# kywind/real2sim-eval

Measured on AMD Instinct MI355X. Metric: sim env-steps/sec (phys+render) per node at 32 envs, higher is better.
Workload: dtype f32

## Files before the change

include/r2s_physics.h:

```cpp
#ifndef R2S_PHYSICS_H
#define R2S_PHYSICS_H

#include <stddef.h>
#include <stdint.h>
#include "r2s_raster.h"

#ifdef __cplusplus
extern "C" {
#endif

typedef struct R2SPhysParams {
    float dt;
    float dashpot_damping;
    float drag_damping;
    float spring_Y_min;
    float spring_Y_max;
    float collision_dist;
    float collide_elas, collide_fric;
    float collide_eef_elas, collide_eef_fric;
    float collide_self_elas, collide_self_fric;
    int32_t reverse_z;
    int32_t self_collision;
    int32_t use_pusher;
    int32_t num_substeps;
// ... 101 lines not shown
    char kernel[192];
} R2SFlavourOut;
int r2s_phys_debug_pick_flavour(const R2SFlavourIn* in, R2SFlavourOut* out);
int r2s_phys_debug_flavour_input(R2SPhys* h, R2SFlavourIn* out);

int r2s_phys_last_flavour_ex(R2SPhys* h, R2SFlavourOut* out);
int r2s_phys_check_fault(R2SPhys* h, r2s_stream_t stream);

int r2s_phys_set_tuning(R2SPhys* h, int chains, int mesh_defer);
int r2s_phys_set_resident(R2SPhys* h, int on);
int r2s_phys_set_pf(R2SPhys* h, int on);
int r2s_phys_side_stream(int32_t k, r2s_stream_t* out);

int r2s_phys_layout_stats(R2SPhys* h, int64_t* out);

void r2s_phys_set_timing(R2SPhys* h, int enable);
int r2s_phys_last_step_ms(R2SPhys* h, float* ms, int32_t* kernels);

#ifdef __cplusplus
}
#endif
#endif
```

real2sim-eval_amd/csrc/physics.hip:

```cpp

#include "r2s_common.h"
#include <rocprim/rocprim.hpp>
#include "../../include/r2s_physics.h"
#include "physics_flavour.h"
#include <algorithm>
#include <array>
#include <climits>
#include <cmath>
#include <cstdlib>
#include <mutex>
#include <vector>
#include <functional>

namespace {

constexpr int SLICE = 64;

constexpr int GROUP = 4;
constexpr int TPB = 256;
constexpr int GRID_DIM = 128;
constexpr int GRID_CELL_BITS = 21;
constexpr float MESH_MAX_DIST = 0.02f;
constexpr float WIND_THRESHOLD = 0.6f;
constexpr float NEAR_PAD = 0.03f;
// ... 1 lines not shown
struct PhysDev {
    int N, E, n_sub;
    int nb, cb;
    int e0, ne;
    const int* slice_off;
    const int* slice_deg;
    const int* slice_int;
    const uint2* adj_idx;
    const float4* adj_k;
    const float4* adj_ir;
    const int* rslice_off;
    const int* rslice_deg;
    const int4* radj;
    const int* halo_off;
    const int* halo_ids;
    const int* perm;
    const int* inv;
    const float* masses;
    const int* masks;
    float dt, dashpot, drag_factor, rf, cd;
    float ce, cf, cee, cef, cse, csf;
    int self_collision, use_pusher;
    const int* coll_num;
    const int* coll_idx;
    int coll_cap;
    size_t par_stride;
    float4* vbc;
    float4* xbc;
    float4* vdef;
    int2* mesh_list;
// ... 103 lines not shown

struct R2SPhys {
    R2SPhysParams prm{};
    int E = 0, N = 0, S = 0, n_slices = 0, ell_len = 0;
    int nb = 0, cb = 0, halo_max = 0;
    int pb = 256, rcap = 1024;
    int coll_cap = 500;
    int words = 0;
    int n_mesh = 0, n_dyn_mesh = 0, nF = 0, nV = 0, n_dyn_pts = 0;
    std::vector<int> h_springs;
    std::vector<float> h_rest;
    std::vector<int> h_adj_spring;
    std::vector<int> h_adj_nbr;
    std::vector<int> h_adj_self;
    std::vector<int> h_adj_loc;
    std::vector<int> h_perm, h_inv, h_slice_off, h_slice_deg, h_rslice_off, h_rslice_deg, h_slice_int;
    std::vector<int> h_radj_spring, h_radj_nbr, h_radj_self;
    std::vector<int> h_mesh_map, h_face_map;
    v2f* xv[2] = {nullptr, nullptr};
    StateM state(int b) const { return {xv[b], (size_t)E * N}; }
    int cur = 0;
    int *d_slice_off = nullptr, *d_slice_deg = nullptr, *d_rslice_off = nullptr, *d_rslice_deg = nullptr, *d_slice_int = nullptr;
    unsigned short* d_adj_idx = nullptr;
    float *d_adj_k = nullptr, *d_adj_ir = nullptr;
    int4* d_radj = nullptr;
    int rell_len = 0;
    int *d_halo_off = nullptr, *d_halo_ids = nullptr, *d_perm = nullptr, *d_inv = nullptr;
    int *d_num_user = nullptr, *d_idx_user = nullptr;
    float* d_masses = nullptr;
    int* d_masks = nullptr;
    int *d_coll_num = nullptr, *d_coll_idx = nullptr, *d_max_count = nullptr;
// ... 84 lines not shown
    hipGraph_t graph_tail[MAX_CHAINS][12] = {};
    hipGraphExec_t graph_exec_tail[MAX_CHAINS][12] = {};
    int graph_head = 64;
    hipEvent_t chain_fork = nullptr, chain_join[MAX_CHAINS] = {};
    bool timing = false;
    hipEvent_t ev0 = nullptr, ev1 = nullptr;
    int last_kernels = 0;
    bool ev_pending = false;

    PhysDev dev() const
    {
        PhysDev p{};
        p.N = N; p.E = E; p.n_sub = prm.num_substeps;
        p.nb = nb; p.cb = cb; p.e0 = 0; p.ne = E;
        p.slice_off = d_slice_off; p.slice_deg = d_slice_deg; p.slice_int = d_slice_int; p.adj_idx = (const uint2*)d_adj_idx; p.adj_k = (const float4*)d_adj_k; p.adj_ir = (const float4*)d_adj_ir; p.rslice_off = d_rslice_off; p.rslice_deg = d_rslice_deg; p.radj = d_radj;
        p.halo_off = d_halo_off; p.halo_ids = d_halo_ids; p.perm = d_perm; p.inv = d_inv;
        p.masses = d_masses; p.masks = d_masks;
        p.dt = prm.dt; p.dashpot = prm.dashpot_damping; p.drag_factor = expf(-prm.dt * prm.drag_damping);
        p.rf = prm.reverse_z ? -1.f : 1.f; p.cd = prm.collision_dist;
        auto cl = [](float x, float lo, float hi) { return std::min(std::max(x, lo), hi); };
        p.ce = cl(prm.collide_elas, 0.f, 1.f); p.cf = cl(prm.collide_fric, 0.f, 2.f);
        p.cee = cl(prm.collide_eef_elas, 0.f, 1.f); p.cef = cl(prm.collide_eef_fric, 0.f, 2.f);
        p.cse = cl(prm.collide_self_elas, 0.f, 1.f); p.csf = cl(prm.collide_self_fric, 0.f, 2.f);
        p.self_collision = prm.self_collision; p.use_pusher = prm.use_pusher;
        p.coll_num = d_coll_num; p.coll_idx = d_coll_idx; p.coll_cap = coll_cap;
        p.vbc = d_vbc; p.xbc = d_xbc; p.par_stride = (size_t)E * N; p.cand_list = d_cand_list; p.cand_count = d_cand_count; p.cand_cnt_env = d_cand_count ? d_cand_count + 4 : nullptr;
        p.pf = 0; p.pf_nfin = 0; p.pf_res = d_pf_res;
        p.mesh_list = d_mesh_list; p.mesh_cnt = d_mesh_cnt; p.mesh_cap = mesh_cap; p.mesh_defer = mesh_defer; p.vdef = d_vdef; p.cand_mark = d_cand_mark; p.mesh_rec = d_mesh_rec; p.rec_cnt = d_rec_cnt; p.mq_hint = d_mq_hint;
        p.lm_c0 = lm[0]; p.lm_nc = lm[1]; p.lm_f0 = lm[2]; p.lm_f1 = lm[3]; p.lm_y = lm[4]; p.lm_mesh = lm[5]; p.lm_slot = lm[6];
        p.n_mesh = n_mesh; p.n_dyn_mesh = n_dyn_mesh; p.nF = nF; p.nV = nV; p.n_dyn_pts = n_dyn_pts;
        p.faces = d_faces; p.mesh_map = d_mesh_map; p.face_map = d_face_map; p.mesh_face_off = d_mesh_face_off;
// ... 503 lines not shown
        auto spread = [](uint64_t v) {
            v &= 0x1fffff; v = (v | v << 32) & 0x1f00000000ffffull; v = (v | v << 16) & 0x1f0000ff0000ffull;
            v = (v | v << 8) & 0x100f00f00f00f00full; v = (v | v << 4) & 0x10c30c30c30c30c3ull; v = (v | v << 2) & 0x1249249249249249ull;
            return v;
        };
        std::vector<std::pair<uint64_t, int>> code(N);
        for (int i = 0; i < N; ++i) {
            uint64_t c = 0;
            for (int k = 0; k < 3; ++k) {
                const double t = (d->init_vertices[3 * i + k] - lo[k]) / ext;
                c |= spread((uint64_t)std::min(1048575.0, std::max(0.0, t * 1048575.0))) << k;
            }
            code[i] = {c, i};
        }
        std::sort(code.begin(), code.end());
        std::vector<int> degree(N, 0);
        for (int sp = 0; sp < S; ++sp) { degree[h->h_springs[2 * sp]]++; degree[h->h_springs[2 * sp + 1]]++; }
        for (int b0 = 0; b0 < N; b0 += PB)
            std::stable_sort(code.begin() + b0, code.begin() + std::min(N, b0 + PB),
                             [&](const std::pair<uint64_t, int>& a, const std::pair<uint64_t, int>& b) { return degree[a.second] > degree[b.second]; });
        for (int i = 0; i < N; ++i) { h->h_perm[i] = code[i].second; h->h_inv[code[i].second] = i; }
    }
    TRY(dev_alloc(&h->d_perm, N)); TRY(dev_alloc(&h->d_inv, N));
    TRY(upload(h->d_perm, h->h_perm.data(), N, s)); TRY(upload(h->d_inv, h->h_inv.data(), N, s));

    std::vector<std::vector<std::pair<int, int>>> adj(N);
    for (int sp = 0; sp < S; ++sp) {
        const int a = h->h_inv[h->h_springs[2 * sp]], b = h->h_inv[h->h_springs[2 * sp + 1]];
        adj[a].push_back({b, sp});
        adj[b].push_back({a, sp});
    }
    for (auto& l : adj) std::sort(l.begin(), l.end());
    h->n_slices = (N + SL - 1) / SL;
    h->nb = (N + PB - 1) / PB;
    h->cb = (h->nb * E + 7) / 8;
    int HALO_CAP = h->rcap - PB;
    if (const char* ev = getenv("R2S_HALO_CAP")) HALO_CAP = std::min(HALO_CAP, std::max(0, atoi(ev)));
    std::vector<int> halo_off(h->nb + 1, 0), halo_ids;
    std::vector<int> slot_of(N, -1);
    std::vector<std::vector<int>> halo_of_block(h->nb);
    h->halo_max = 0;
    for (int b = 0; b < h->nb; ++b) {
        std::vector<std::pair<int, int>> cnt;
        {
            std::vector<int> refs;
            for (int i = b * PB; i < std::min(N, (b + 1) * PB); ++i)
                for (auto& nb : adj[i]) if (nb.first / PB != b) refs.push_back(nb.first);
            std::sort(refs.begin(), refs.end());
            for (size_t a = 0; a < refs.size();) {
                size_t e2 = a;
                while (e2 < refs.size() && refs[e2] == refs[a]) ++e2;
                cnt.push_back({-(int)(e2 - a), refs[a]});
                a = e2;
            }
        }
        std::sort(cnt.begin(), cnt.end());
        if ((int)cnt.size() > HALO_CAP) cnt.resize(HALO_CAP);
        std::vector<int>& hl = halo_of_block[b];
        for (auto& c : cnt) hl.push_back(c.second);
        std::sort(hl.begin(), hl.end());
        halo_off[b + 1] = halo_off[b] + (int)hl.size();
        halo_ids.insert(halo_ids.end(), hl.begin(), hl.end());
        h->halo_max = std::max(h->halo_max, (int)hl.size());
    }
    std::vector<std::vector<std::array<int, 3>>> loc(N), rem(N);
    for (int b = 0; b < h->nb; ++b) {
        const std::vector<int>& hl = halo_of_block[b];
        for (size_t k = 0; k < hl.size(); ++k) slot_of[hl[k]] = PB + (int)k;
        for (int i = b * PB; i < std::min(N, (b + 1) * PB); ++i)
            for (auto& nb : adj[i]) {
                const int j = nb.first;
                if (j / PB == b) loc[i].push_back({j, nb.second, j % PB});
                else if (slot_of[j] >= 0) loc[i].push_back({j, nb.second, slot_of[j]});
                else rem[i].push_back({j, nb.second, -1});
            }
        for (size_t k = 0; k < hl.size(); ++k) slot_of[hl[k]] = -1;
    }
    h->h_slice_int.assign(h->n_slices, 0);
    if (PB == SL)
        for (int b = 0; b < h->nb; ++b) {
            int imax = 0;
            for (int i = b * PB; i < std::min(N, (b + 1) * PB); ++i) {
                std::stable_partition(loc[i].begin(), loc[i].end(), [&](const std::array<int, 3>& a) { return a[2] < PB; });
                int ni = 0;
                for (auto& a : loc[i]) ni += a[2] < PB;
                imax = std::max(imax, ni);
            }
            imax = (imax + GROUP - 1) / GROUP * GROUP;
            h->h_slice_int[b] = imax;
            for (int i = b * PB; i < std::min(N, (b + 1) * PB); ++i) {
                int ni = 0;
                for (auto& a : loc[i]) ni += a[2] < PB;
                loc[i].insert(loc[i].begin() + ni, (size_t)(imax - ni), std::array<int, 3>{i, -1, i % PB});
// ... 1080 lines not shown
    R2S_HIP_TRY(hipGetLastError());
    return R2S_OK;
}

int r2s_phys_layout_stats(R2SPhys* h, int64_t* out )
{
    if (!h || !out) return R2S_ERR_INVALID;
    int64_t real = 0, fallback = 0;
    for (int t = 0; t < h->ell_len; ++t) if (h->h_adj_spring[t] >= 0) ++real;
    for (int t = 0; t < h->rell_len; ++t) if (h->h_radj_spring[t] >= 0) { ++real; ++fallback; }
    out[0] = h->nb; out[1] = h->halo_max; out[2] = h->ell_len + h->rell_len; out[3] = real; out[4] = fallback;
    out[5] = (int64_t)h->rcap * 24; out[6] = h->chains(); out[7] = h->cb;
    return R2S_OK;
}

void r2s_phys_set_timing(R2SPhys* h, int enable) { if (h) h->timing = enable != 0; }

int r2s_phys_last_step_ms(R2SPhys* h, float* ms, int32_t* kernels)
{
    if (!h || !ms || !h->ev_pending) return R2S_ERR_INVALID;
    R2S_HIP_TRY(hipEventSynchronize(h->ev1));
    R2S_HIP_TRY(hipEventElapsedTime(ms, h->ev0, h->ev1));
    if (kernels) *kernels = h->last_kernels;
    return R2S_OK;
}

}
```

real2sim-eval_amd/csrc/physics_resident.h:

```cpp

constexpr int RES_THREADS = 512;
constexpr int RES_NG = 2;
constexpr unsigned RES_SPIN_LIMIT = 1u << 21;
constexpr int RES_AUX_SC1 = 16;
#ifndef R2S_RES_AUXLD
#define R2S_RES_AUXLD (16 | (int)0x80000000)
#endif
#ifndef R2S_RES_PRE
#define R2S_RES_PRE 2
#endif
#ifndef R2S_RES_DELAY
#define R2S_RES_DELAY 0
#endif
constexpr int RES_AUX_LOAD = R2S_RES_AUXLD;
constexpr int RES_PRE = R2S_RES_PRE;

struct GroupRecs { v2f xy[GROUP], zz[GROUP], vv[GROUP]; };
template <int RCAP>
__device__ __forceinline__ void group_read(const AdjGroup& g, const __attribute__((address_space(3))) char* win, GroupRecs& r)
{
    typedef __attribute__((address_space(3))) const v2f lds_f2;
    const unsigned off[GROUP] = {g.idx.x & 0xffffu, g.idx.x >> 16, g.idx.y & 0xffffu, g.idx.y >> 16};
#pragma unroll
    for (int u = 0; u < GROUP; ++u) {
// ... 88 lines not shown
    const bool own = p.srv_own != 0;
    const int pl = r * 64 + lane;
    const unsigned xn = ((unsigned)p.N + 7u) & ~7u, xe = (unsigned)e * 6u * xn, xb = 3u * xn * 16u;
    const __amdgpu_buffer_rsrc_t rx = __builtin_amdgcn_make_buffer_rsrc(p.xch, 0, 0x7fffffff, 0x00020000);
    unsigned noff = 0, roff = 0;
    float sk = 0.f, sa = 0.f, m1 = 1.f, inv_m1 = 1.f;
    bool live = false;
    if (own) {
        const int b = i / SLICE, l = i - b * SLICE;
        const int srow = p.slice_off[b] / GROUP, nslot = p.slice_deg[b];
        if (pl < nslot) {
            const size_t el = (size_t)(srow + (pl / GROUP) * SLICE + l) * GROUP + (size_t)(pl % GROUP);
            const unsigned off = ((const unsigned short*)p.adj_idx)[el];
            sk = ((const float*)p.adj_k)[el]; sa = ((const float*)p.adj_ir)[el];
            const int w = (int)(off >> 3);
            const int gid = w < SLICE ? b * SLICE + w : p.halo_ids[p.halo_off[b] + (w - SLICE)];
            live = gid != i && (sk != 0.f || sa != 0.f);
            noff = (xe + (unsigned)gid) * 16u;
            roff = ((unsigned)e * (unsigned)p.N + (unsigned)gid) * (unsigned)SRV_REC + (unsigned)SRV_RES;
        }
        m1 = p.masses[i]; inv_m1 = 1.0f / m1;
    }
    f3 sx = mk(0.f, 0.f, 0.f), sv = sx;
    bool have = false;
    const unsigned k_first = k;
#ifdef R2S_PHASE_PROBE
    long long sp_acc[6] = {0, 0, 0, 0, 0, 0}, sp_t = (long long)wall_clock64();
#define R2S_SSTAMP(kk) do { const long long now_ = (long long)wall_clock64(); sp_acc[kk] += now_ - sp_t; sp_t = now_; } while (0)
#else
#define R2S_SSTAMP(kk) do { } while (0)
#endif
// ... 127 lines not shown
    const unsigned xn = ((unsigned)p.N + 7u) & ~7u;
    const unsigned xe = (unsigned)e * 6u * xn, xb = 3u * xn * 16u;
    const __amdgpu_buffer_rsrc_t rx = __builtin_amdgcn_make_buffer_rsrc(p.xch, 0, 0x7fffffff, 0x00020000);
    __attribute__((address_space(3))) char* win_w = (__attribute__((address_space(3))) char*)win_s;
    const __attribute__((address_space(3))) char* win = win_w;
    const bool finisher = wave < (n_steps == 1 ? 1 : 3);

    const int h0 = p.halo_off[b], nh = p.halo_off[b + 1] - h0, nt = 3 * nh;
    unsigned t_off[KT], t_lds[KT], pend0 = 0;
#pragma unroll
    for (int k = 0; k < KT; ++k) {
        const int t = tid + RES_THREADS * k;
        t_off[k] = 0; t_lds[k] = 0;
        if (t < nt) {
            const int pl = t / nh, r = t - pl * nh;
            const int hid = p.halo_ids[h0 + r];
            t_off[k] = (xe + (unsigned)pl * xn + (unsigned)hid) * 16u;
            t_lds[k] = (unsigned)(pl * (RCAP + 1) + B + r) * 8u;
            pend0 |= 1u << k;
            win_s[pl * (RCAP + 1) + B + r] = xv_in.p[st_at(xv_in.n, eb + (size_t)hid, pl)];
        }
    }
    if (wave < 3) win_s[wave * (RCAP + 1) + lane] = xv_in.p[st_at(xv_in.n, eb + (size_t)ic, wave)];
    const int srow = __builtin_amdgcn_readfirstlane(p.slice_off[b] / GROUP);
    const int ng = __builtin_amdgcn_readfirstlane(p.slice_deg[b] / GROUP), gi = __builtin_amdgcn_readfirstlane(p.slice_int[b] / GROUP);
    const int n_own = gi > wave ? (gi - wave + NW - 1) / NW : 0;
    const int n_all = ng > wave ? (ng - wave + NW - 1) / NW : 0, n_halo = n_all - n_own;
    AdjGroup ag_own[RES_NG], ag_halo[RES_NG];
#pragma unroll
    for (int j = 0; j < RES_NG; ++j) {
        ag_own[j].idx = make_uint2(0u, 0u); ag_own[j].k = make_float4(0.f, 0.f, 0.f, 0.f); ag_own[j].a = ag_own[j].k;
// ... 561 lines not shown
```

real2sim-eval_amd/csrc/physics_substep.h:

```cpp

typedef unsigned v4u __attribute__((ext_vector_type(4)));
constexpr unsigned PF_SENT = 0x7fc5e7a1u;
constexpr int PF_LINE = 128;
constexpr int PF_AUX_STORE = 16;
constexpr int PF_AUX_LOAD = 16 | (int)0x80000000;
__device__ __forceinline__ void resident_fault(const PhysDev& p, int code, int item, int k, unsigned a, unsigned b, unsigned c, unsigned d, unsigned e2, unsigned f)
{
    if (!p.fault) return;
    if (atomicCAS(p.fault, 0, code) == 0) {
        int* w = p.fault + 3;
        w[0] = code; w[1] = item; w[2] = k; w[3] = (int)a; w[4] = (int)b; w[5] = (int)c; w[6] = (int)d; w[7] = (int)e2; w[8] = (int)f;
    }
}
__device__ __forceinline__ bool pf_pending(v2f a) { return __float_as_uint(a.x) == PF_SENT && __float_as_uint(a.y) == PF_SENT; }
__device__ __forceinline__ void pf_mark(StateM s, size_t i)
{
    const v2f w = {__uint_as_float(PF_SENT), __uint_as_float(PF_SENT)};
    s.p[st_at(s.n, i, 0)] = w; s.p[st_at(s.n, i, 1)] = w; s.p[st_at(s.n, i, 2)] = w;
}
__device__ __forceinline__ void pf_store(const PhysDev& p, size_t ei, f3 x, f3 v, unsigned tag)
{
    const __amdgpu_buffer_rsrc_t r = __builtin_amdgcn_make_buffer_rsrc(p.pf_res, 0, 0x7fffffff, 0x00020000);
    const unsigned off = (unsigned)ei * (unsigned)PF_LINE;
    const v4u w0 = {__float_as_uint(x.x), tag, __float_as_uint(x.y), tag}, w1 = {__float_as_uint(x.z), tag, __float_as_uint(v.z), tag},
// ... 75 lines not shown
#ifdef R2S_WIN16
        typedef float v4f_ __attribute__((ext_vector_type(4)));
        typedef __attribute__((address_space(3))) const v4f_ lds_f4;
        const v4f_ xz = *(lds_f4*)(win + 2u * off[u]);
        const v2f vxy = *(lds_f2*)(win + off[u] + 2 * (RCAP * 8 + 8));
        spring_term((v2f){xz.x, xz.y}, xz.z, vxy, xz.w, xi, vi, k[u], a[u], p.dashpot, fxy, fz);
#else
        const v2f xy = *(lds_f2*)(win + off[u]);
        const v2f zz = *(lds_f2*)(win + off[u] + PLANE1<RCAP>());
        const v2f vxy = *(lds_f2*)(win + off[u] + PLANE2<RCAP>());
        spring_term(xy, zz.x, vxy, zz.y, xi, vi, k[u], a[u], p.dashpot, fxy, fz);
#endif
    }
}

template <int RCAP>
__device__ __forceinline__ f3 spring_force_lds(const PhysDev& p, const StateC xv,
                                               const __attribute__((address_space(3))) char* win, size_t env_base, int sl, int ln, f3 xi,
                                               f3 vi, int srow, int ngroups, AdjGroup g0, int pf_step = -1)
{
    v2f fxy = {0.f, 0.f};
    float fz = 0.f;
    AdjGroup a = g0, b = g0;
    int g = 0;
    for (; g + 2 <= ngroups; g += 2) {
        b = adj_load(p, srow + (g + 1) * SLICE, ln);
        spring_group<RCAP>(p, a, win, xi, vi, fxy, fz);
        a = adj_load(p, srow + min(g + 2, ngroups - 1) * SLICE, ln);
        spring_group<RCAP>(p, b, win, xi, vi, fxy, fz);
    }
    if (g < ngroups) spring_group<RCAP>(p, a, win, xi, vi, fxy, fz);
    const int4* __restrict__ ra = p.radj + p.rslice_off[sl] + ln;
    const int rdeg = p.rslice_deg[sl];
    for (int n = 0; n < rdeg; ++n) {
        const int4 en = ra[n * SLICE];
        const size_t gi = env_base + (size_t)en.x;
        v2f jxy = xv.p[st_at(xv.n, gi, 0)], jz = xv.p[st_at(xv.n, gi, 1)], jv = xv.p[st_at(xv.n, gi, 2)];
        if (pf_step >= 0 && pf_pending(jxy)) pf_wait(p, gi, pf_step, -1, jxy, jz, jv);
        spring_term(jxy, jz.x, jv, jz.y, xi, vi, __int_as_float(en.y), __int_as_float(en.z), p.dashpot, fxy, fz);
    }
    return {fxy.x, fxy.y, fz};
}

#pragma clang fp contract(off)

__device__ __forceinline__ float mesh_margin(const PhysDev& p, int m)
{
    return (p.mesh_kind[m] & 2) ? MESH_MAX_DIST : ((m < p.n_dyn_mesh && !p.use_pusher) ? 0.005f : 0.001f);
}
__device__ __forceinline__ bool mesh_need(const PhysDev& p, int e, int step, f3 next_x, float pad, bool& near, const float* staged = nullptr)
{
    bool need = false;
    near = false;
    for (int m = 0; m < p.n_mesh; ++m) {
        const float* bb = staged ? staged + 6 * m
                        : m < p.n_dyn_mesh ? p.aabb_dyn + (((size_t)e * p.n_sub + step) * p.n_dyn_mesh + m) * 6
// ... 195 lines not shown
            v1 = v_normal_new + v_tao * a;
            toi = -(x_z - 0.f) / v_z;
        } else {
            v1 = v;
            toi = 0.f;
        }
        const f3 xn = x + v * toi + v1 * (p.dt - toi);
        if (PFOUT) { if (store) pf_store(p, eb + (size_t)i, xn, v1, (unsigned)step + 1u); }
        else if (store && (!KEEP || xv_out.p != nullptr)) st_store(xv_out, eb + i, xn, v1);
        if (KEEP) { keep->x = xn; keep->v = v1; }
        return true;
    }
    return false;
}

#ifdef R2S_PHASE_PROBE
__device__ long long g_phase_probe[8192 * 4];
#define R2S_STAMP(k) do { if (threadIdx.x == 0 && blockIdx.x < 8192) g_phase_probe[blockIdx.x * 4 + (k)] = (long long)wall_clock64(); } while (0)
extern "C" int r2s_phys_debug_phase_probe(long long* out, int n)
{
    return (int)hipMemcpyFromSymbol(out, HIP_SYMBOL(g_phase_probe), sizeof(long long) * (size_t)n * 4);
}
#else
#define R2S_STAMP(k) do { } while (0)
#endif

template <int B, int RCAP, bool SELF, int MESH, bool PF = false, bool EXTWIN = false>
__device__ __forceinline__ void substep_body(const PhysDev& p, const StateC xv_in, const StateM xv_out, int step,
                                             int write_forces, int bid, __attribute__((address_space(3))) v2f* win_ext = nullptr)
{
    static_assert(B % SLICE == 0 && RCAP >= B && RCAP * 8 <= 65536, "window offsets are u16 bytes");
    __shared__ __attribute__((aligned(16))) v2f win_own[EXTWIN ? 1 : 3 * (RCAP + 1)];
    __attribute__((address_space(3))) v2f* const win_s = EXTWIN ? win_ext : (__attribute__((address_space(3))) v2f*)win_own;
    const int xcd = bid & 7, q = bid >> 3;
    const int item = xcd * p.cb + q;
    if (q >= p.cb || item >= p.nb * p.ne) return;
// ... 3 lines not shown
    const int b = item / p.ne, e = p.e0 + (item - b * p.ne);
#endif
    R2S_STAMP(0);
    const int tid = threadIdx.x;
    const int lane = tid & 63;
    const int i = b * B + tid;
    const bool valid = i < p.N;
    const size_t eb = (size_t)e * p.N;
    const int ic = min(i, p.N - 1);
    const int sl = __builtin_amdgcn_readfirstlane(ic / SLICE);
    const int srow = __builtin_amdgcn_readfirstlane(p.slice_off[sl] / GROUP);
    const int ngroups = __builtin_amdgcn_readfirstlane(p.slice_deg[sl] / GROUP);
    AdjGroup g0;
    g0.idx = make_uint2(0u, 0u); g0.k = make_float4(0.f, 0.f, 0.f, 0.f); g0.a = g0.k;
    if (ngroups > 0) g0 = adj_load(p, srow, lane);
    constexpr int K = (RCAP + B - 1) / B;
#ifndef R2S_STAGE_BATCH
#define R2S_STAGE_BATCH 4
#endif
#ifndef R2S_STAGE64
#define R2S_STAGE64 2
#endif
    constexpr int KB = B == 64 ? (R2S_STAGE64 < K ? R2S_STAGE64 : K) : ((R2S_STAGE_BATCH > 0 && R2S_STAGE_BATCH < K) ? R2S_STAGE_BATCH : K);
    const int h0 = p.halo_off[b], per_env = B + (p.halo_off[b + 1] - h0);
    v2f own_a = {0.f, 0.f}, own_b = own_a, own_c = own_a;
#pragma unroll
    for (int k0 = 0; k0 < K; k0 += KB) {
        int part[KB];
#pragma unroll
        for (int k = 0; k < KB; ++k) {
            const int r = tid + (k0 + k) * B;
            part[k] = (k0 + k >= K) ? p.N : (r < B ? i : (r < per_env ? p.halo_ids[h0 + r - B] : p.N));
        }
        v2f qa[KB], qb[KB], qc[KB];
#pragma unroll
        for (int k = 0; k < KB; ++k) {
            const size_t g = eb + (size_t)min(part[k], p.N - 1);
            if (part[k] < p.N) { qa[k] = xv_in.p[st_at(xv_in.n, g, 0)]; qb[k] = xv_in.p[st_at(xv_in.n, g, 1)]; qc[k] = xv_in.p[st_at(xv_in.n, g, 2)]; }
            else { qa[k] = (v2f){0.f, 0.f}; qb[k] = qa[k]; qc[k] = qa[k]; }
        }
        if (PF) {
#pragma unroll
            for (int k = 0; k < KB; ++k)
                if (part[k] < p.N && pf_pending(qa[k])) pf_wait(p, eb + (size_t)part[k], step, item, qa[k], qb[k], qc[k]);
        }
#pragma unroll
        for (int k = 0; k < KB; ++k) {
            const int r = tid + (k0 + k) * B;
            if (r < RCAP && part[k] < p.N) {
#ifdef R2S_WIN16
                win_s[2 * r] = qa[k];
                win_s[2 * r + 1] = qb[k];
                win_s[2 * (RCAP + 1) + r] = qc[k];
#else
                win_s[r] = qa[k];
                win_s[RCAP + 1 + r] = qb[k];
                win_s[2 * (RCAP + 1) + r] = qc[k];
#endif
            }
        }
        if (k0 == 0) { own_a = qa[0]; own_b = qb[0]; own_c = qc[0]; }
    }
    __syncthreads();
    R2S_STAMP(1);
    const f3 x0 = mk(own_a.x, own_a.y, own_b.x), v0 = mk(own_c.x, own_c.y, own_b.y);
    const float m1 = p.masses[ic];

    const __attribute__((address_space(3))) char* win = (const __attribute__((address_space(3))) char*)win_s;
    f3 v = vel_update(p, v0, spring_force_lds<RCAP>(p, xv_in, win, eb, sl, lane, x0, v0, srow, ngroups, g0, PF ? step : -1), m1);
#ifdef R2S_PHASE_PROBE
    if (v.x == 1.2345e33f) return;
#endif
    R2S_STAMP(2);

    bool fin = valid;
    const bool rec_mode = PF && MESH != 0 && p.mesh_rec != nullptr && (p.mesh_defer || MESH == 2);
    int tag_ncand = 0;
    if (SELF) {
        const int ncand = valid ? p.coll_num[eb + i] : 0;
        if (ncand > 0) {
            const size_t po = par_off(p, step);
            p.vbc[po + eb + i] = make_float4(v.x, v.y, v.z, 0.f);
            p.xbc[po + eb + i] = make_float4(x0.x, x0.y, x0.z, 0.f);
            fin = false;
            if (rec_mode) tag_ncand = ncand;
            else if (MESH != 0 && (p.mesh_defer || MESH == 2)) {
                bool near;
                if (mesh_need(p, e, step, x0 + v * p.dt, 0.002f, near)) {
// ... 23 lines not shown
        const unsigned long long qm = __builtin_amdgcn_ballot_w64(need);
        if (qm && lane == __builtin_ctzll(qm)) p.fault[1] = 1;
        int slot = 0;
        if (need) { slot = mesh_rec_reserve(p, e, step); fin = false; }
        done = finish_wave<MESH, false, 2>(p, e, i, eb, step, write_forces, x0, v, fin, xv_out, nullptr, nullptr, nullptr, nullptr, true, nullptr R2S_QP_ARG);
        if (need) {
            if (slot < p.N) {
                mesh_rec_write(p, e, step, slot, i, tag_ncand, x0, v);
                if (tag_ncand > 0) p.cand_mark[par_off(p, step) + eb + i] = step + 1;
            } else
                resident_fault(p, 8, item, step, (unsigned)(eb + i), (unsigned)slot, 0u, 0u, 0u, 0u);
        }
    } else
        done = finish_wave<MESH, MESH != 0>(p, e, i, eb, step, write_forces, x0, v, fin, xv_out, nullptr, nullptr, nullptr, nullptr, true, nullptr R2S_QP_ARG);
    if (PF && valid && !done) pf_mark(xv_out, eb + i);
    R2S_STAMP(3);
}

template <int B, int RCAP, bool SELF, int MESH>
__global__ void __launch_bounds__(B, (B == 256 ? 6 : 1)) k_substep(const PhysDev p, const StateC xv_in, const StateM xv_out, int step,
                                               int write_forces)
{
    substep_body<B, RCAP, SELF, MESH>(p, xv_in, xv_out, step, write_forces, (int)blockIdx.x);
}
```

real2sim-eval_amd/r2s_hip/physics.py:

```python
from __future__ import annotations

import ctypes as C
from typing import Optional

import numpy as np
import torch

from . import _lib
from ._lib import check, cur_stream


class R2SPhysParams(C.Structure):
    _fields_ = [
        ("dt", C.c_float), ("dashpot_damping", C.c_float), ("drag_damping", C.c_float), ("spring_Y_min", C.c_float),
        ("spring_Y_max", C.c_float), ("collision_dist", C.c_float), ("collide_elas", C.c_float), ("collide_fric", C.c_float),
        ("collide_eef_elas", C.c_float), ("collide_eef_fric", C.c_float), ("collide_self_elas", C.c_float),
        ("collide_self_fric", C.c_float), ("reverse_z", C.c_int32), ("self_collision", C.c_int32), ("use_pusher", C.c_int32),
        ("num_substeps", C.c_int32),
    ]


class R2SPhysDesc(C.Structure):
    _fields_ = [
        ("params", R2SPhysParams), ("n_env", C.c_int32), ("num_object_points", C.c_int32), ("num_springs", C.c_int32),
# ... 43 lines not shown
    vp, i32 = C.c_void_p, C.c_int
    L.r2s_phys_create.restype = i32
    L.r2s_phys_create.argtypes = [C.POINTER(R2SPhysDesc), C.POINTER(vp), vp]
    L.r2s_phys_destroy.restype = None
    L.r2s_phys_destroy.argtypes = [vp]
    for name, args in dict(
        r2s_phys_set_state=[vp, vp, vp, vp], r2s_phys_get_state=[vp, vp, vp, vp], r2s_phys_create_resting_case=[vp, vp],
        r2s_phys_update_collision_graph=[vp, vp], r2s_phys_set_mesh_interactive=[vp, vp, vp, vp, vp, vp],
        r2s_phys_step=[vp, i32, i32, vp], r2s_phys_collision_forces=[vp, C.POINTER(vp), C.POINTER(C.c_int32)],
        r2s_phys_mesh_maps=[vp, vp, vp], r2s_phys_collision_lists=[vp, C.POINTER(vp), C.POINTER(vp), C.POINTER(C.c_int32)],
        r2s_phys_collision_max_count=[vp, C.POINTER(C.c_int32), vp], r2s_phys_set_spring_Y=[vp, vp, vp],
        r2s_phys_set_eef_table=[vp, C.c_int32, vp, vp, C.c_float, vp], r2s_phys_set_eef_motion=[vp, vp, vp, vp, vp, vp, vp],
        r2s_phys_eef_state=[vp, C.POINTER(vp), C.POINTER(vp)], r2s_phys_reset_envs=[vp, vp, vp], r2s_phys_set_state_envs=[vp, vp, vp, vp, vp], r2s_phys_create_resting_case_envs=[vp, vp, vp], r2s_phys_mesh_motion=[vp, C.POINTER(vp), C.POINTER(vp), C.POINTER(vp), C.POINTER(vp)],
        r2s_phys_set_collision_lists=[vp, vp, vp, vp], r2s_phys_contact_stats=[vp, C.POINTER(C.c_int32), C.POINTER(vp)],
        r2s_phys_last_flavour=[vp, C.POINTER(C.c_int32)], r2s_phys_deferred_counts=[vp, vp, vp], r2s_phys_tagged_count=[vp, C.POINTER(C.c_int32), vp], r2s_phys_log_contacts=[vp, vp, vp], r2s_phys_set_tuning=[vp, i32, i32], r2s_phys_set_resident=[vp, i32], r2s_phys_set_pf=[vp, i32], r2s_phys_set_static_mesh_points=[vp, vp, C.c_int32, vp, vp], r2s_phys_side_stream=[i32, C.POINTER(vp)],
        r2s_phys_set_params=[vp, C.POINTER(R2SPhysParams), vp], r2s_phys_debug_pick_flavour=[C.POINTER(R2SFlavourIn), C.POINTER(R2SFlavourOut)], r2s_phys_debug_flavour_input=[vp, C.POINTER(R2SFlavourIn)], r2s_phys_last_flavour_ex=[vp, C.POINTER(R2SFlavourOut)], r2s_phys_check_fault=[vp, vp], r2s_phys_layout_stats=[vp, C.POINTER(C.c_int64)], r2s_phys_last_step_ms=[vp, C.POINTER(C.c_float), C.POINTER(C.c_int32)],
    ).items():
        fn = getattr(L, name)
        fn.restype = i32
        fn.argtypes = args
    L.r2s_phys_set_timing.restype = None
    L.r2s_phys_set_timing.argtypes = [vp, i32]
    _bound = True
    return L


def _np(a, dtype):
    if isinstance(a, torch.Tensor):
        a = a.detach().cpu().numpy()
    return np.ascontiguousarray(np.asarray(a, dtype=dtype))

# ... 316 lines not shown

    def set_params(self, **kw):
        for k, v in kw.items():
            if k not in self._FLOAT_PARAMS:
                raise ValueError(f"{k!r} is not a settable scalar parameter (structural fields are fixed at construction)")
            setattr(self.params, k, float(np.asarray(v.detach().cpu() if isinstance(v, torch.Tensor) else v, np.float32).reshape(-1)[0]))
        with torch.cuda.device(self.device):
            check(_bind().r2s_phys_set_params(self._h, C.byref(self.params), self._s()), "r2s_phys_set_params")

    def layout_stats(self):
        a = (C.c_int64 * 8)()
        check(_bind().r2s_phys_layout_stats(self._h, a), "r2s_phys_layout_stats")
        k = ["blocks", "halo_max", "ell_slots", "neighbour_slots", "fallback_slots", "lds_bytes", "chains", "blocks_per_xcd"]
        return dict(zip(k, [int(v) for v in a]))

    def set_timing(self, on: bool):
        _bind().r2s_phys_set_timing(self._h, int(on))

    def last_step_ms(self):
        ms, k = C.c_float(), C.c_int32()
        check(_bind().r2s_phys_last_step_ms(self._h, C.byref(ms), C.byref(k)), "r2s_phys_last_step_ms")
        return float(ms.value), int(k.value)
```

Measured before the change: 1832.

## Overlap halo staging with interior spring forces using padded halo layout

The substep kernel now stages only each block's own particles into LDS, computes the spring groups whose neighbours are all block-local, and only then loads halo particles and finishes the remaining groups after a second barrier. Host layout code sorts particles by in-block degree, pads each slice's adjacency so interior springs come first (slice_int), and stores halo ids in a fixed-stride per-block array. The goal is to hide the latency of global halo loads behind interior spring work. In exchange it adds an extra __syncthreads, padding slots in the ELL layout, and a debug ELL export entry point.

```diff
diff --git a/include/r2s_physics.h b/include/r2s_physics.h
--- a/include/r2s_physics.h
+++ b/include/r2s_physics.h
@@ -139,6 +139,9 @@
 
 int r2s_phys_layout_stats(R2SPhys* h, int64_t* out);
 
+int r2s_phys_debug_ell(R2SPhys* h, int64_t* n, int32_t* slice_off, int32_t* slice_deg, int32_t* slice_int, int32_t* adj_spring, int32_t* adj_loc,
+                       int32_t* radj_spring, int32_t* halo_ids);
+
 void r2s_phys_set_timing(R2SPhys* h, int enable);
 int r2s_phys_last_step_ms(R2SPhys* h, float* ms, int32_t* kernels);
 
diff --git a/real2sim-eval_amd/csrc/physics.hip b/real2sim-eval_amd/csrc/physics.hip
--- a/real2sim-eval_amd/csrc/physics.hip
+++ b/real2sim-eval_amd/csrc/physics.hip
@@ -39,6 +39,7 @@
     const int4* radj;
     const int* halo_off;
     const int* halo_ids;
+    int halo_stride;
     const int* perm;
     const int* inv;
     const float* masses;
@@ -172,7 +173,7 @@
     std::vector<int> h_adj_nbr;
     std::vector<int> h_adj_self;
     std::vector<int> h_adj_loc;
-    std::vector<int> h_perm, h_inv, h_slice_off, h_slice_deg, h_rslice_off, h_rslice_deg, h_slice_int;
+    std::vector<int> h_perm, h_inv, h_slice_off, h_slice_deg, h_rslice_off, h_rslice_deg, h_slice_int, h_halo_ids;
     std::vector<int> h_radj_spring, h_radj_nbr, h_radj_self;
     std::vector<int> h_mesh_map, h_face_map;
     v2f* xv[2] = {nullptr, nullptr};
@@ -287,7 +288,7 @@
         p.N = N; p.E = E; p.n_sub = prm.num_substeps;
         p.nb = nb; p.cb = cb; p.e0 = 0; p.ne = E;
         p.slice_off = d_slice_off; p.slice_deg = d_slice_deg; p.slice_int = d_slice_int; p.adj_idx = (const uint2*)d_adj_idx; p.adj_k = (const float4*)d_adj_k; p.adj_ir = (const float4*)d_adj_ir; p.rslice_off = d_rslice_off; p.rslice_deg = d_rslice_deg; p.radj = d_radj;
-        p.halo_off = d_halo_off; p.halo_ids = d_halo_ids; p.perm = d_perm; p.inv = d_inv;
+        p.halo_off = d_halo_off; p.halo_ids = d_halo_ids; p.halo_stride = rcap - pb; p.perm = d_perm; p.inv = d_inv;
         p.masses = d_masses; p.masks = d_masks;
         p.dt = prm.dt; p.dashpot = prm.dashpot_damping; p.drag_factor = expf(-prm.dt * prm.drag_damping);
         p.rf = prm.reverse_z ? -1.f : 1.f; p.cd = prm.collision_dist;
@@ -821,11 +822,20 @@
             code[i] = {c, i};
         }
         std::sort(code.begin(), code.end());
-        std::vector<int> degree(N, 0);
+        std::vector<int> degree(N, 0), own_degree(N, 0);
         for (int sp = 0; sp < S; ++sp) { degree[h->h_springs[2 * sp]]++; degree[h->h_springs[2 * sp + 1]]++; }
+        if (PB != SL) {
+            std::vector<int> blk(N);
+            for (int i = 0; i < N; ++i) blk[code[i].second] = i / PB;
+            for (int sp = 0; sp < S; ++sp) {
+                const int a = h->h_springs[2 * sp], b = h->h_springs[2 * sp + 1];
+                if (blk[a] == blk[b]) { own_degree[a]++; own_degree[b]++; }
+            }
+        }
         for (int b0 = 0; b0 < N; b0 += PB)
-            std::stable_sort(code.begin() + b0, code.begin() + std::min(N, b0 + PB),
-                             [&](const std::pair<uint64_t, int>& a, const std::pair<uint64_t, int>& b) { return degree[a.second] > degree[b.second]; });
+            std::stable_sort(code.begin() + b0, code.begin() + std::min(N, b0 + PB), [&](const std::pair<uint64_t, int>& a, const std::pair<uint64_t, int>& b) {
+                return degree[a.second] != degree[b.second] ? degree[a.second] > degree[b.second] : own_degree[a.second] > own_degree[b.second];
+            });
         for (int i = 0; i < N; ++i) { h->h_perm[i] = code[i].second; h->h_inv[code[i].second] = i; }
     }
     TRY(dev_alloc(&h->d_perm, N)); TRY(dev_alloc(&h->d_inv, N));
@@ -843,7 +853,10 @@
     h->cb = (h->nb * E + 7) / 8;
     int HALO_CAP = h->rcap - PB;
     if (const char* ev = getenv("R2S_HALO_CAP")) HALO_CAP = std::min(HALO_CAP, std::max(0, atoi(ev)));
-    std::vector<int> halo_off(h->nb + 1, 0), halo_ids;
+    const int HS = h->rcap - PB;
+    std::vector<int> halo_off(h->nb + 1, 0);
+    std::vector<int>& halo_ids = h->h_halo_ids;
+    halo_ids.assign((size_t)h->nb * HS, N);
     std::vector<int> slot_of(N, -1);
     std::vector<std::vector<int>> halo_of_block(h->nb);
     h->halo_max = 0;
@@ -867,7 +880,7 @@
         for (auto& c : cnt) hl.push_back(c.second);
         std::sort(hl.begin(), hl.end());
         halo_off[b + 1] = halo_off[b] + (int)hl.size();
-        halo_ids.insert(halo_ids.end(), hl.begin(), hl.end());
+        std::copy(hl.begin(), hl.end(), halo_ids.begin() + (size_t)b * HS);
         h->halo_max = std::max(h->halo_max, (int)hl.size());
     }
     std::vector<std::vector<std::array<int, 3>>> loc(N), rem(N);
@@ -884,6 +897,31 @@
         for (size_t k = 0; k < hl.size(); ++k) slot_of[hl[k]] = -1;
     }
     h->h_slice_int.assign(h->n_slices, 0);
+    if (PB != SL)
+        for (int sl = 0; sl < h->n_slices; ++sl) {
+            const int i0 = sl * SL, i1 = std::min(N, (sl + 1) * SL);
+            std::vector<int> own(i1 - i0);
+            int dmax = 0;
+            for (int i = i0; i < i1; ++i) {
+                std::stable_partition(loc[i].begin(), loc[i].end(), [&](const std::array<int, 3>& a) { return a[2] < PB; });
+                int ni = 0;
+                for (auto& a : loc[i]) ni += a[2] < PB;
+                own[i - i0] = ni;
+                dmax = std::max(dmax, (int)loc[i].size());
+            }
+            dmax = (dmax + GROUP - 1) / GROUP * GROUP;
+            int t = dmax;
+            auto fits = [&](int tt) {
+                for (int i = i0; i < i1; ++i)
+                    if (own[i - i0] < tt && (int)loc[i].size() + tt - own[i - i0] > dmax) return false;
+                return true;
+            };
+            while (t > 0 && !fits(t)) t -= GROUP;
+            h->h_slice_int[sl] = t;
+            for (int i = i0; i < i1; ++i)
+                if (own[i - i0] < t && (int)loc[i].size() > own[i - i0])
+                    loc[i].insert(loc[i].begin() + own[i - i0], (size_t)(t - own[i - i0]), std::array<int, 3>{i, -1, i % PB});
+        }
     if (PB == SL)
         for (int b = 0; b < h->nb; ++b) {
             int imax = 0;
@@ -1994,6 +2032,17 @@
     return R2S_OK;
 }
 
+int r2s_phys_debug_ell(R2SPhys* h, int64_t* n, int32_t* slice_off, int32_t* slice_deg, int32_t* slice_int, int32_t* adj_spring, int32_t* adj_loc,
+                       int32_t* radj_spring, int32_t* halo_ids)
+{
+    if (!h || !n) return R2S_ERR_INVALID;
+    n[0] = h->n_slices; n[1] = h->ell_len; n[2] = h->rell_len; n[3] = h->nb; n[4] = h->rcap - h->pb;
+    auto put = [](int32_t* dst, const std::vector<int>& src) { if (dst) std::copy(src.begin(), src.end(), dst); };
+    put(slice_off, h->h_slice_off); put(slice_deg, h->h_slice_deg); put(slice_int, h->h_slice_int);
+    put(adj_spring, h->h_adj_spring); put(adj_loc, h->h_adj_loc); put(radj_spring, h->h_radj_spring); put(halo_ids, h->h_halo_ids);
+    return R2S_OK;
+}
+
 void r2s_phys_set_timing(R2SPhys* h, int enable) { if (h) h->timing = enable != 0; }
 
 int r2s_phys_last_step_ms(R2SPhys* h, float* ms, int32_t* kernels)
diff --git a/real2sim-eval_amd/csrc/physics_resident.h b/real2sim-eval_amd/csrc/physics_resident.h
--- a/real2sim-eval_amd/csrc/physics_resident.h
+++ b/real2sim-eval_amd/csrc/physics_resident.h
@@ -126,7 +126,7 @@
             const unsigned off = ((const unsigned short*)p.adj_idx)[el];
             sk = ((const float*)p.adj_k)[el]; sa = ((const float*)p.adj_ir)[el];
             const int w = (int)(off >> 3);
-            const int gid = w < SLICE ? b * SLICE + w : p.halo_ids[p.halo_off[b] + (w - SLICE)];
+            const int gid = w < SLICE ? b * SLICE + w : p.halo_ids[(size_t)b * p.halo_stride + (w - SLICE)];
             live = gid != i && (sk != 0.f || sa != 0.f);
             noff = (xe + (unsigned)gid) * 16u;
             roff = ((unsigned)e * (unsigned)p.N + (unsigned)gid) * (unsigned)SRV_REC + (unsigned)SRV_RES;
@@ -284,7 +284,7 @@
         t_off[k] = 0; t_lds[k] = 0;
         if (t < nt) {
             const int pl = t / nh, r = t - pl * nh;
-            const int hid = p.halo_ids[h0 + r];
+            const int hid = p.halo_ids[(size_t)b * p.halo_stride + r];
             t_off[k] = (xe + (unsigned)pl * xn + (unsigned)hid) * 16u;
             t_lds[k] = (unsigned)(pl * (RCAP + 1) + B + r) * 8u;
             pend0 |= 1u << k;
diff --git a/real2sim-eval_amd/csrc/physics_substep.h b/real2sim-eval_amd/csrc/physics_substep.h
--- a/real2sim-eval_amd/csrc/physics_substep.h
+++ b/real2sim-eval_amd/csrc/physics_substep.h
@@ -113,22 +113,25 @@
     }
 }
 
-template <int RCAP>
-__device__ __forceinline__ f3 spring_force_lds(const PhysDev& p, const StateC xv,
-                                               const __attribute__((address_space(3))) char* win, size_t env_base, int sl, int ln, f3 xi,
-                                               f3 vi, int srow, int ngroups, AdjGroup g0, int pf_step = -1)
-{
-    v2f fxy = {0.f, 0.f};
-    float fz = 0.f;
-    AdjGroup a = g0, b = g0;
-    int g = 0;
-    for (; g + 2 <= ngroups; g += 2) {
+template <int RCAP, bool NEXT>
+__device__ __forceinline__ void spring_range(const PhysDev& p, const __attribute__((address_space(3))) char* win, int ln, f3 xi, f3 vi, int srow,
+                                              int ngroups, int g, int ge, AdjGroup& a, v2f& fxy, float& fz)
+{
+    AdjGroup b = a;
+    for (; g + 2 <= ge; g += 2) {
         b = adj_load(p, srow + (g + 1) * SLICE, ln);
         spring_group<RCAP>(p, a, win, xi, vi, fxy, fz);
         a = adj_load(p, srow + min(g + 2, ngroups - 1) * SLICE, ln);
         spring_group<RCAP>(p, b, win, xi, vi, fxy, fz);
     }
-    if (g < ngroups) spring_group<RCAP>(p, a, win, xi, vi, fxy, fz);
+    if (g < ge) {
+        spring_group<RCAP>(p, a, win, xi, vi, fxy, fz);
+        if (NEXT) a = adj_load(p, srow + min(g + 1, ngroups - 1) * SLICE, ln);
+    }
+}
+__device__ __forceinline__ void spring_remote(const PhysDev& p, const StateC xv, size_t env_base, int sl, int ln, f3 xi, f3 vi, v2f& fxy, float& fz,
+                                              int pf_step = -1)
+{
     const int4* __restrict__ ra = p.radj + p.rslice_off[sl] + ln;
     const int rdeg = p.rslice_deg[sl];
     for (int n = 0; n < rdeg; ++n) {
@@ -138,7 +141,6 @@
         if (pf_step >= 0 && pf_pending(jxy)) pf_wait(p, gi, pf_step, -1, jxy, jz, jv);
         spring_term(jxy, jz.x, jv, jz.y, xi, vi, __int_as_float(en.y), __int_as_float(en.z), p.dashpot, fxy, fz);
     }
-    return {fxy.x, fxy.y, fz};
 }
 
 #pragma clang fp contract(off)
@@ -364,12 +366,52 @@
     return false;
 }
 
+template <int HB> struct HaloBatch { int part[HB]; v2f qa[HB], qb[HB], qc[HB]; };
+template <int B, int KH, int HB>
+__device__ __forceinline__ void halo_load(const PhysDev& p, const StateC xv_in, const int* __restrict__ hrow, size_t eb, int k0, HaloBatch<HB>& h)
+{
+#pragma unroll
+    for (int k = 0; k < HB; ++k) h.part[k] = (k0 + k < KH) ? hrow[(k0 + k) * B] : p.N;
+#pragma unroll
+    for (int k = 0; k < HB; ++k) {
+        const size_t g = eb + (size_t)min(h.part[k], p.N - 1);
+        if (h.part[k] < p.N) { h.qa[k] = xv_in.p[st_at(xv_in.n, g, 0)]; h.qb[k] = xv_in.p[st_at(xv_in.n, g, 1)]; h.qc[k] = xv_in.p[st_at(xv_in.n, g, 2)]; }
+        else { h.qa[k] = (v2f){0.f, 0.f}; h.qb[k] = h.qa[k]; h.qc[k] = h.qa[k]; }
+    }
+}
+template <int RCAP>
+__device__ __forceinline__ void win_store(__attribute__((address_space(3))) v2f* win_s, int r, v2f a, v2f b, v2f c)
+{
+#ifdef R2S_WIN16
+    win_s[2 * r] = a;
+    win_s[2 * r + 1] = b;
+    win_s[2 * (RCAP + 1) + r] = c;
+#else
+    win_s[r] = a;
+    win_s[RCAP + 1 + r] = b;
+    win_s[2 * (RCAP + 1) + r] = c;
+#endif
+}
+template <int B, int RCAP, int KH, int HB, bool PF>
+__device__ __forceinline__ void halo_store(const PhysDev& p, __attribute__((address_space(3))) v2f* win_s, size_t eb, int tid, int step, int item, int k0, HaloBatch<HB>& h)
+{
+    if (PF) {
+#pragma unroll
+        for (int k = 0; k < HB; ++k)
+            if (h.part[k] < p.N && pf_pending(h.qa[k])) pf_wait(p, eb + (size_t)h.part[k], step, item, h.qa[k], h.qb[k], h.qc[k]);
+    }
+#pragma unroll
+    for (int k = 0; k < HB; ++k)
+        if (k0 + k < KH && h.part[k] < p.N) win_store<RCAP>(win_s, tid + (1 + k0 + k) * B, h.qa[k], h.qb[k], h.qc[k]);
+}
+
 #ifdef R2S_PHASE_PROBE
-__device__ long long g_phase_probe[8192 * 4];
-#define R2S_STAMP(k) do { if (threadIdx.x == 0 && blockIdx.x < 8192) g_phase_probe[blockIdx.x * 4 + (k)] = (long long)wall_clock64(); } while (0)
+constexpr int PROBE_STAMPS = 6;
+__device__ long long g_phase_probe[8192 * PROBE_STAMPS];
+#define R2S_STAMP(k) do { if (threadIdx.x == 0 && blockIdx.x < 8192) g_phase_probe[blockIdx.x * PROBE_STAMPS + (k)] = (long long)wall_clock64(); } while (0)
 extern "C" int r2s_phys_debug_phase_probe(long long* out, int n)
 {
-    return (int)hipMemcpyFromSymbol(out, HIP_SYMBOL(g_phase_probe), sizeof(long long) * (size_t)n * 4);
+    return (int)hipMemcpyFromSymbol(out, HIP_SYMBOL(g_phase_probe), sizeof(long long) * (size_t)n * PROBE_STAMPS);
 }
 #else
 #define R2S_STAMP(k) do { } while (0)
@@ -403,64 +445,47 @@
     AdjGroup g0;
     g0.idx = make_uint2(0u, 0u); g0.k = make_float4(0.f, 0.f, 0.f, 0.f); g0.a = g0.k;
     if (ngroups > 0) g0 = adj_load(p, srow, lane);
-    constexpr int K = (RCAP + B - 1) / B;
+    constexpr int K = (RCAP + B - 1) / B, KH = K - 1, HS = RCAP - B;
 #ifndef R2S_STAGE_BATCH
 #define R2S_STAGE_BATCH 4
 #endif
 #ifndef R2S_STAGE64
 #define R2S_STAGE64 2
 #endif
-    constexpr int KB = B == 64 ? (R2S_STAGE64 < K ? R2S_STAGE64 : K) : ((R2S_STAGE_BATCH > 0 && R2S_STAGE_BATCH < K) ? R2S_STAGE_BATCH : K);
-    const int h0 = p.halo_off[b], per_env = B + (p.halo_off[b + 1] - h0);
+    constexpr int HB0 = B == 64 ? R2S_STAGE64 : R2S_STAGE_BATCH - 1, HB = HB0 < 1 ? 1 : (HB0 > KH ? KH : HB0);
+    static_assert(KH >= 1 && HS % B == 0, "whole halo rounds");
+    const int gint = min(__builtin_amdgcn_readfirstlane(p.slice_int[sl] / GROUP), ngroups);
     v2f own_a = {0.f, 0.f}, own_b = own_a, own_c = own_a;
-#pragma unroll
-    for (int k0 = 0; k0 < K; k0 += KB) {
-        int part[KB];
-#pragma unroll
-        for (int k = 0; k < KB; ++k) {
-            const int r = tid + (k0 + k) * B;
-            part[k] = (k0 + k >= K) ? p.N : (r < B ? i : (r < per_env ? p.halo_ids[h0 + r - B] : p.N));
-        }
-        v2f qa[KB], qb[KB], qc[KB];
-#pragma unroll
-        for (int k = 0; k < KB; ++k) {
-            const size_t g = eb + (size_t)min(part[k], p.N - 1);
-            if (part[k] < p.N) { qa[k] = xv_in.p[st_at(xv_in.n, g, 0)]; qb[k] = xv_in.p[st_at(xv_in.n, g, 1)]; qc[k] = xv_in.p[st_at(xv_in.n, g, 2)]; }
-            else { qa[k] = (v2f){0.f, 0.f}; qb[k] = qa[k]; qc[k] = qa[k]; }
-        }
-        if (PF) {
-#pragma unroll
-            for (int k = 0; k < KB; ++k)
-                if (part[k] < p.N && pf_pending(qa[k])) pf_wait(p, eb + (size_t)part[k], step, item, qa[k], qb[k], qc[k]);
-        }
-#pragma unroll
-        for (int k = 0; k < KB; ++k) {
-            const int r = tid + (k0 + k) * B;
-            if (r < RCAP && part[k] < p.N) {
-#ifdef R2S_WIN16
-                win_s[2 * r] = qa[k];
-                win_s[2 * r + 1] = qb[k];
-                win_s[2 * (RCAP + 1) + r] = qc[k];
-#else
-                win_s[r] = qa[k];
-                win_s[RCAP + 1 + r] = qb[k];
-                win_s[2 * (RCAP + 1) + r] = qc[k];
-#endif
-            }
-        }
-        if (k0 == 0) { own_a = qa[0]; own_b = qb[0]; own_c = qc[0]; }
-    }
+    if (valid) { own_a = xv_in.p[st_at(xv_in.n, eb + (size_t)i, 0)]; own_b = xv_in.p[st_at(xv_in.n, eb + (size_t)i, 1)]; own_c = xv_in.p[st_at(xv_in.n, eb + (size_t)i, 2)]; }
+    HaloBatch<HB> hq;
+    const int* __restrict__ hrow = p.halo_ids + (size_t)b * HS + tid;
+    halo_load<B, KH, HB>(p, xv_in, hrow, eb, 0, hq);
+    if (PF && valid && pf_pending(own_a)) pf_wait(p, eb + (size_t)i, step, item, own_a, own_b, own_c);
+    if (valid) win_store<RCAP>(win_s, tid, own_a, own_b, own_c);
     __syncthreads();
     R2S_STAMP(1);
     const f3 x0 = mk(own_a.x, own_a.y, own_b.x), v0 = mk(own_c.x, own_c.y, own_b.y);
     const float m1 = p.masses[ic];
 
     const __attribute__((address_space(3))) char* win = (const __attribute__((address_space(3))) char*)win_s;
-    f3 v = vel_update(p, v0, spring_force_lds<RCAP>(p, xv_in, win, eb, sl, lane, x0, v0, srow, ngroups, g0, PF ? step : -1), m1);
+    v2f fxy = {0.f, 0.f};
+    float fz = 0.f;
+    spring_range<RCAP, true>(p, win, lane, x0, v0, srow, ngroups, 0, gint, g0, fxy, fz);
+    R2S_STAMP(2);
+#pragma unroll
+    for (int k0 = 0; k0 < KH; k0 += HB) {
+        if (k0 > 0) halo_load<B, KH, HB>(p, xv_in, hrow, eb, k0, hq);
+        halo_store<B, RCAP, KH, HB, PF>(p, win_s, eb, tid, step, item, k0, hq);
+    }
+    __syncthreads();
+    R2S_STAMP(3);
+    spring_range<RCAP, false>(p, win, lane, x0, v0, srow, ngroups, gint, ngroups, g0, fxy, fz);
+    spring_remote(p, xv_in, eb, sl, lane, x0, v0, fxy, fz, PF ? step : -1);
+    f3 v = vel_update(p, v0, mk(fxy.x, fxy.y, fz), m1);
 #ifdef R2S_PHASE_PROBE
     if (v.x == 1.2345e33f) return;
 #endif
-    R2S_STAMP(2);
+    R2S_STAMP(4);
 
     bool fin = valid;
     const bool rec_mode = PF && MESH != 0 && p.mesh_rec != nullptr && (p.mesh_defer || MESH == 2);
@@ -514,7 +539,7 @@
     } else
         done = finish_wave<MESH, MESH != 0>(p, e, i, eb, step, write_forces, x0, v, fin, xv_out, nullptr, nullptr, nullptr, nullptr, true, nullptr R2S_QP_ARG);
     if (PF && valid && !done) pf_mark(xv_out, eb + i);
-    R2S_STAMP(3);
+    R2S_STAMP(5);
 }
 
 template <int B, int RCAP, bool SELF, int MESH>
diff --git a/real2sim-eval_amd/r2s_hip/physics.py b/real2sim-eval_amd/r2s_hip/physics.py
--- a/real2sim-eval_amd/r2s_hip/physics.py
+++ b/real2sim-eval_amd/r2s_hip/physics.py
@@ -81,7 +81,7 @@
         r2s_phys_eef_state=[vp, C.POINTER(vp), C.POINTER(vp)], r2s_phys_reset_envs=[vp, vp, vp], r2s_phys_set_state_envs=[vp, vp, vp, vp, vp], r2s_phys_create_resting_case_envs=[vp, vp, vp], r2s_phys_mesh_motion=[vp, C.POINTER(vp), C.POINTER(vp), C.POINTER(vp), C.POINTER(vp)],
         r2s_phys_set_collision_lists=[vp, vp, vp, vp], r2s_phys_contact_stats=[vp, C.POINTER(C.c_int32), C.POINTER(vp)],
         r2s_phys_last_flavour=[vp, C.POINTER(C.c_int32)], r2s_phys_deferred_counts=[vp, vp, vp], r2s_phys_tagged_count=[vp, C.POINTER(C.c_int32), vp], r2s_phys_log_contacts=[vp, vp, vp], r2s_phys_set_tuning=[vp, i32, i32], r2s_phys_set_resident=[vp, i32], r2s_phys_set_pf=[vp, i32], r2s_phys_set_static_mesh_points=[vp, vp, C.c_int32, vp, vp], r2s_phys_side_stream=[i32, C.POINTER(vp)],
-        r2s_phys_set_params=[vp, C.POINTER(R2SPhysParams), vp], r2s_phys_debug_pick_flavour=[C.POINTER(R2SFlavourIn), C.POINTER(R2SFlavourOut)], r2s_phys_debug_flavour_input=[vp, C.POINTER(R2SFlavourIn)], r2s_phys_last_flavour_ex=[vp, C.POINTER(R2SFlavourOut)], r2s_phys_check_fault=[vp, vp], r2s_phys_layout_stats=[vp, C.POINTER(C.c_int64)], r2s_phys_last_step_ms=[vp, C.POINTER(C.c_float), C.POINTER(C.c_int32)],
+        r2s_phys_set_params=[vp, C.POINTER(R2SPhysParams), vp], r2s_phys_debug_pick_flavour=[C.POINTER(R2SFlavourIn), C.POINTER(R2SFlavourOut)], r2s_phys_debug_flavour_input=[vp, C.POINTER(R2SFlavourIn)], r2s_phys_last_flavour_ex=[vp, C.POINTER(R2SFlavourOut)], r2s_phys_check_fault=[vp, vp], r2s_phys_layout_stats=[vp, C.POINTER(C.c_int64)], r2s_phys_debug_ell=[vp, C.POINTER(C.c_int64)] + [vp] * 7, r2s_phys_last_step_ms=[vp, C.POINTER(C.c_float), C.POINTER(C.c_int32)],
     ).items():
         fn = getattr(L, name)
         fn.restype = i32
@@ -428,6 +428,17 @@
         k = ["blocks", "halo_max", "ell_slots", "neighbour_slots", "fallback_slots", "lds_bytes", "chains", "blocks_per_xcd"]
         return dict(zip(k, [int(v) for v in a]))
 
+    def debug_ell(self):
+        n = (C.c_int64 * 5)()
+        check(_bind().r2s_phys_debug_ell(self._h, n, None, None, None, None, None, None, None), "r2s_phys_debug_ell")
+        ns, nl, nr, nb, hs = (int(v) for v in n)
+        shapes = dict(slice_off=ns, slice_deg=ns, slice_int=ns, adj_spring=nl, adj_loc=nl, radj_spring=nr, halo_ids=nb * hs)
+        out = {k: np.zeros(max(v, 1), np.int32) for k, v in shapes.items()}
+        check(_bind().r2s_phys_debug_ell(self._h, n, *[out[k].ctypes.data_as(C.c_void_p) for k in shapes]), "r2s_phys_debug_ell")
+        out = {k: out[k][:v] for k, v in shapes.items()}
+        out["halo_ids"] = out["halo_ids"].reshape(nb, hs)
+        return out
+
     def set_timing(self, on: bool):
         _bind().r2s_phys_set_timing(self._h, int(on))
 
```

New measurement: 1791. 0.977x the previous value.
